# sisinflab/elliot

Measured on NVIDIA H100. Metric: bpr_triples_per_sec, higher is better.
Workload: dtype f32

## Files before the change

elliot_b200/csrc/bpr_train.cu:

```cuda
#include <cooperative_groups.h>
#include <cub/cub.cuh>
#include <stdlib.h>

#include <type_traits>

#include "bpr_update.cuh"

namespace eb {

struct HogwildParams {
    float *U, *V, *b;
    int ld;
    const int32_t *tu, *ti, *tj;
    int64_t n;
    BprHyper hp;
    double *loss;
    int32_t n_users, n_items;
    const int64_t *indptr;
    const int32_t *indices;
    uint64_t seed, first;
    int32_t *out_u, *out_i, *out_j;
    float *Vp[EB_MAX_PEERS], *bp[EB_MAX_PEERS];
    ShardMap shards;
    const uint32_t *filter;
    int filter_log2bits;
    const uint64_t *packed;
    int bits_u, bits_i;
    int no_item_updates;
    const int32_t *order;
};

__device__ __forceinline__ void sample_user(const HogwildParams &p, int64_t t, uint32_t (&r)[4], int &u, int64_t &beg, int &len) {
    Philox::gen(p.seed, p.first + (uint64_t)t, 0u, r);
    u = (int)bounded(r[0], (uint32_t)p.n_users);
    beg = __ldg(p.indptr + u);
    int64_t end = __ldg(p.indptr + u + 1);
    len = (int)(end - beg);
    uint32_t attempt = 0;
    while (len == 0 || len >= p.n_items) {
        Philox::gen(p.seed, p.first + (uint64_t)t, ++attempt | 0x80000000u, r);
        u = (int)bounded(r[0], (uint32_t)p.n_users);
        beg = __ldg(p.indptr + u); end = __ldg(p.indptr + u + 1); len = (int)(end - beg);
    }
}

__device__ __forceinline__ void sample_triple(const HogwildParams &p, int64_t t, int &u, int &i, int &j) {
    uint32_t r[4];
    int64_t beg;
    int len;
    sample_user(p, t, r, u, beg, len);
    uint32_t attempt = 0;
    const int32_t *row = p.indices + beg;
    int cand = (int)bounded(r[2], (uint32_t)p.n_items);
    const bool maybe = p.filter ? bloom_maybe(p.filter + ((int64_t)u << (p.filter_log2bits - 5)), p.filter_log2bits, (uint32_t)cand) : true;
    i = __ldg(row + bounded(r[1], (uint32_t)len));
    if (!maybe || !contains_sorted(row, len, cand)) { j = cand; return; }
    cand = (int)bounded(r[3], (uint32_t)p.n_items);
    attempt = 0;
    int q = 4;
    while (contains_sorted(row, len, cand) && attempt < 16u) {
        if (q == 4) { Philox::gen(p.seed, p.first + (uint64_t)t, ++attempt, r); q = 0; }
        cand = (int)bounded(r[q++], (uint32_t)p.n_items);
    }
    if (attempt >= 16u && contains_sorted(row, len, cand)) {
        Philox::gen(p.seed, p.first + (uint64_t)t, 0x40000000u, r);
        const uint32_t rank = bounded(r[0], (uint32_t)(p.n_items - len));
        int lo = 0, hi = len;
        while (lo < hi) {
            const int mid = (lo + hi) >> 1;
            if ((uint32_t)(__ldg(row + mid) - mid) > rank) hi = mid; else lo = mid + 1;
        }
        cand = (int)rank + lo;
    }
    j = cand;
}

template <bool SAMPLE>
__device__ __forceinline__ void fetch_triple(const HogwildParams &p, int64_t t, int &u, int &i, int &j) {
    if (SAMPLE) {
        sample_triple(p, t, u, i, j);
        if (p.out_u) { p.out_u[t] = u; p.out_i[t] = i; p.out_j[t] = j; }
    } else if (p.packed) {
        const uint64_t w = __ldg(p.packed + t);
        u = (int)(w & ((1ull << p.bits_u) - 1));
        i = (int)((w >> p.bits_u) & ((1ull << p.bits_i) - 1));
        j = (int)(w >> (p.bits_u + p.bits_i));
    } else {
        u = __ldg(p.tu + t); i = __ldg(p.ti + t); j = __ldg(p.tj + t);
    }
}

template <bool PEER>
__device__ __forceinline__ void item_row(const HogwildParams &p, int i, float *&row, float *&bias) {
    if constexpr (PEER) {
        int o, l;
        p.shards.locate(i, o, l);
        row = p.Vp[o] + (int64_t)l * p.ld; bias = p.bp[o] + l;
    } else {
        row = p.V + (int64_t)i * p.ld; bias = p.b + i;
    }
}

template <int VPL>
struct Rows {
    float4 u[VPL], vi[VPL], vj[VPL];
    float bi, bj;
};

template <int DP, bool SAMPLE, bool ATOMIC, bool PEER, bool ROUNDS = false>
__global__ void __launch_bounds__(256) bpr_hogwild_kernel(const HogwildParams p) {
    static_assert(!ROUNDS || (ATOMIC && !PEER), "deterministic rounds: local tables, atomic updates");
    constexpr int NV = DP / 4;
    constexpr int G = NV >= 32 ? 32 : NV;
    constexpr int VPL = NV / G;
    const int lane = threadIdx.x & 31;
    const int gl = lane % G;
    const int gbase = lane - gl;
    const int64_t warp_id = ((int64_t)blockIdx.x * blockDim.x + threadIdx.x) >> 5;
    const int64_t nwarps = ((int64_t)gridDim.x * blockDim.x) >> 5;
    const int64_t ld = p.ld;
    float loss_acc = 0.f;

    auto load_rows = [&](Rows<VPL> &r, int u, int i, int j) {
        if (u >= 0) {
            float *ri, *rj, *bi, *bj;
            item_row<PEER>(p, i, ri, bi); item_row<PEER>(p, j, rj, bj);
            const float4 *pu = reinterpret_cast<const float4 *>(p.U + (int64_t)u * ld);
            const float4 *pi = reinterpret_cast<const float4 *>(ri);
            const float4 *pj = reinterpret_cast<const float4 *>(rj);
#pragma unroll
            for (int v = 0; v < VPL; v++) {
                r.u[v] = pu[v * G + gl];
                r.vi[v] = PEER ? ld_sys_v4(pi + v * G + gl) : pi[v * G + gl];
                r.vj[v] = PEER ? ld_sys_v4(pj + v * G + gl) : pj[v * G + gl];
            }
            r.bi = *bi;
            r.bj = *bj;
        }
    };

    const int64_t n_tiles = (p.n + 31) / 32;
    const int64_t tile_end = ROUNDS ? (n_tiles + nwarps - 1) / nwarps * nwarps : n_tiles;
    for (int64_t tile = warp_id; tile < tile_end; tile += nwarps) {
        const int64_t t = tile * 32 + lane;
        int u = -1, i = 0, j = 0;
        if (t < p.n) fetch_triple<SAMPLE>(p, t, u, i, j);
        constexpr int UNR = G >= 4 ? 4 : G;
#pragma unroll 1
        for (int s0 = 0; s0 < G; s0 += UNR) {
            Rows<VPL> rw[UNR];
            int tu_[UNR], ti_[UNR], tj_[UNR];
#pragma unroll
            for (int q = 0; q < UNR; q++) {
                tu_[q] = __shfl_sync(0xffffffffu, u, gbase + s0 + q);
                ti_[q] = __shfl_sync(0xffffffffu, i, gbase + s0 + q);
                tj_[q] = __shfl_sync(0xffffffffu, j, gbase + s0 + q);
                load_rows(rw[q], tu_[q], ti_[q], tj_[q]);
            }
            if constexpr (ROUNDS) {
#pragma unroll
                for (int q = 0; q < UNR; q++) {
                    Rows<VPL> &cur = rw[q];
                    float part = 0.f;
                    if (tu_[q] >= 0) {
#pragma unroll
                        for (int v = 0; v < VPL; v++) part += bpr_partial_dot(cur.u[v], cur.vi[v], cur.vj[v]);
                    }
                    part = group_sum<G>(part);
                    if (tu_[q] >= 0) {
                        const float z = bpr_sigmoid_loss(part + (cur.bi - cur.bj), loss_acc, gl);
#pragma unroll
                        for (int v = 0; v < VPL; v++) {
                            float4 du, di, dj;
                            bpr_row_deltas(cur.u[v], cur.vi[v], cur.vj[v], z, p.hp, du, di, dj);
                            cur.u[v] = du; cur.vi[v] = di; cur.vj[v] = dj;
                        }
                        float dbi, dbj;
                        bpr_bias_deltas(z, cur.bi, cur.bj, p.hp, dbi, dbj);
                        cur.bi = dbi; cur.bj = dbj;
                    }
                }
                cooperative_groups::this_grid().sync();
#pragma unroll
                for (int q = 0; q < UNR; q++) {
                    if (tu_[q] < 0) continue;
                    float *pu = p.U + (int64_t)tu_[q] * ld, *pi, *pj, *pbi, *pbj;
                    item_row<PEER>(p, ti_[q], pi, pbi); item_row<PEER>(p, tj_[q], pj, pbj);
#pragma unroll
                    for (int v = 0; v < VPL; v++) {
                        const int e = (v * G + gl) * 4;
                        red_add_v4(pu + e, rw[q].u[v]);
                        red_add_v4(pi + e, rw[q].vi[v]);
                        red_add_v4(pj + e, rw[q].vj[v]);
                    }
                    if (gl == 0) { red_add_f32(pbi, rw[q].bi); red_add_f32(pbj, rw[q].bj); }
                }
                cooperative_groups::this_grid().sync();
                continue;
            }
#pragma unroll
            for (int q = 0; q < UNR; q++) {
                const Rows<VPL> &cur = rw[q];
                const int cu = tu_[q], ci = ti_[q], cj = tj_[q];
                float part = 0.f;
                if (cu >= 0) {
#pragma unroll
                    for (int v = 0; v < VPL; v++) part += bpr_partial_dot(cur.u[v], cur.vi[v], cur.vj[v]);
                }
                part = group_sum<G>(part);
                if (cu >= 0) {
                    const float z = bpr_sigmoid_loss(part + (cur.bi - cur.bj), loss_acc, gl);
                    float *pu = p.U + (int64_t)cu * ld, *pi, *pj, *pbi, *pbj;
                    item_row<PEER>(p, ci, pi, pbi); item_row<PEER>(p, cj, pj, pbj);
#pragma unroll
                    for (int v = 0; v < VPL; v++) {
                        const float4 a = cur.u[v], vi = cur.vi[v], vj = cur.vj[v];
                        float4 du, di, dj;
                        bpr_row_deltas(a, vi, vj, z, p.hp, du, di, dj);
                        const int e = (v * G + gl) * 4;
                        if (PEER) {
                            red_add_v4(pu + e, du);
                            if (!p.no_item_updates) {
                                red_add_v4_sys(pi + e, di);
                                red_add_v4_sys(pj + e, dj);
                            }
                        } else if (ATOMIC) {
                            red_add_v4(pu + e, du);
                            red_add_v4(pi + e, di);
                            red_add_v4(pj + e, dj);
                        } else {
                            *reinterpret_cast<float4 *>(pu + e) = make_float4(a.x + du.x, a.y + du.y, a.z + du.z, a.w + du.w);
                            *reinterpret_cast<float4 *>(pi + e) = make_float4(vi.x + di.x, vi.y + di.y, vi.z + di.z, vi.w + di.w);
                            *reinterpret_cast<float4 *>(pj + e) = make_float4(vj.x + dj.x, vj.y + dj.y, vj.z + dj.z, vj.w + dj.w);
                        }
                    }
                    if (gl == 0) {
                        float dbi, dbj;
                        bpr_bias_deltas(z, cur.bi, cur.bj, p.hp, dbi, dbj);
                        if (PEER) { red_add_f32_sys(pbi, dbi); red_add_f32_sys(pbj, dbj); }
                        else if (ATOMIC) { red_add_f32(pbi, dbi); red_add_f32(pbj, dbj); }
                        else { *pbi = cur.bi + dbi; *pbj = cur.bj + dbj; }
                    }
                }
            }
        }
    }
    if (p.loss) {
#pragma unroll
        for (int off = 16; off > 0; off >>= 1) loss_acc += __shfl_xor_sync(0xffffffffu, loss_acc, off);
        if (lane == 0 && loss_acc != 0.f) atomicAdd(p.loss, (double)loss_acc);
    }
}

__global__ void __launch_bounds__(256) user_key_kernel(const HogwildParams p, uint32_t *__restrict__ key, int32_t *__restrict__ val) {
    int64_t t = (int64_t)blockIdx.x * blockDim.x + threadIdx.x;
    const int64_t stride = (int64_t)gridDim.x * blockDim.x;
    for (; t < p.n; t += stride) {
        uint32_t r[4];
        int u, len;
        int64_t beg;
        sample_user(p, t, r, u, beg, len);
        key[t] = (uint32_t)u; val[t] = (int32_t)t;
    }
}

template <int DP, bool ATOMIC>
__global__ void __launch_bounds__(256) bpr_grouped_kernel(const HogwildParams p) {
    constexpr int NV = DP / 4;
    constexpr int G = NV >= 32 ? 32 : NV;
    constexpr int VPL = NV / G;
    constexpr int UNR = G >= 4 ? 4 : G;
    const int lane = threadIdx.x & 31;
    const int gl = lane % G;
    const int gbase = lane - gl;
    const int64_t warp_id = ((int64_t)blockIdx.x * blockDim.x + threadIdx.x) >> 5;
    const int64_t nwarps = ((int64_t)gridDim.x * blockDim.x) >> 5;
    const int64_t ld = p.ld;
    float loss_acc = 0.f;

    const int64_t n_tiles = (p.n + 31) / 32;
    for (int64_t tile = warp_id; tile < n_tiles; tile += nwarps) {
        const int64_t pos = tile * 32 + lane;
        int u = -1, i = 0, j = 0;
        if (pos < p.n) fetch_triple<true>(p, __ldg(p.order + pos), u, i, j);
        int cu = -1;
        float4 cur[VPL], acc[VPL];
        auto flush = [&]() {
            float *pu = p.U + (int64_t)cu * ld;
#pragma unroll
            for (int v = 0; v < VPL; v++) {
                float *e = pu + (v * G + gl) * 4;
                if (ATOMIC) red_add_v4(e, acc[v]);
                else *reinterpret_cast<float4 *>(e) = cur[v];
            }
        };
#pragma unroll 1
        for (int s0 = 0; s0 < G; s0 += UNR) {
            Rows<VPL> rw[UNR];
            int tu_[UNR], ti_[UNR], tj_[UNR];
#pragma unroll
            for (int q = 0; q < UNR; q++) {
                tu_[q] = __shfl_sync(0xffffffffu, u, gbase + s0 + q);
                ti_[q] = __shfl_sync(0xffffffffu, i, gbase + s0 + q);
                tj_[q] = __shfl_sync(0xffffffffu, j, gbase + s0 + q);
                if (tu_[q] >= 0) {
                    if (tu_[q] != (q == 0 ? cu : tu_[q - 1])) {
                        const float4 *pu = reinterpret_cast<const float4 *>(p.U + (int64_t)tu_[q] * ld);
#pragma unroll
                        for (int v = 0; v < VPL; v++) rw[q].u[v] = pu[v * G + gl];
                    }
                    const float4 *pi = reinterpret_cast<const float4 *>(p.V + (int64_t)ti_[q] * ld);
                    const float4 *pj = reinterpret_cast<const float4 *>(p.V + (int64_t)tj_[q] * ld);
#pragma unroll
                    for (int v = 0; v < VPL; v++) { rw[q].vi[v] = pi[v * G + gl]; rw[q].vj[v] = pj[v * G + gl]; }
                    rw[q].bi = p.b[ti_[q]];
                    rw[q].bj = p.b[tj_[q]];
                }
            }
#pragma unroll
            for (int q = 0; q < UNR; q++) {
                const Rows<VPL> &nx = rw[q];
                const int qu = tu_[q], qi = ti_[q], qj = tj_[q];
                const bool start = qu != cu;
                if (start) {
                    if (cu >= 0) flush();
                    cu = qu;
#pragma unroll
                    for (int v = 0; v < VPL; v++) cur[v] = nx.u[v];
                }
                float part = 0.f;
                if (qu >= 0) {
#pragma unroll
                    for (int v = 0; v < VPL; v++) part += bpr_partial_dot(cur[v], nx.vi[v], nx.vj[v]);
                }
                part = group_sum<G>(part);
                if (qu >= 0) {
                    const float z = bpr_sigmoid_loss(part + (nx.bi - nx.bj), loss_acc, gl);
                    float *pi = p.V + (int64_t)qi * ld, *pj = p.V + (int64_t)qj * ld;
#pragma unroll
                    for (int v = 0; v < VPL; v++) {
                        const float4 a = cur[v], vi = nx.vi[v], vj = nx.vj[v];
                        float4 du, di, dj;
                        bpr_row_deltas(a, vi, vj, z, p.hp, du, di, dj);
                        cur[v] = make_float4(a.x + du.x, a.y + du.y, a.z + du.z, a.w + du.w);
                        acc[v] = start ? du : make_float4(acc[v].x + du.x, acc[v].y + du.y, acc[v].z + du.z, acc[v].w + du.w);
                        const int e = (v * G + gl) * 4;
                        if (ATOMIC) {
                            red_add_v4(pi + e, di);
                            red_add_v4(pj + e, dj);
                        } else {
                            *reinterpret_cast<float4 *>(pi + e) = make_float4(vi.x + di.x, vi.y + di.y, vi.z + di.z, vi.w + di.w);
                            *reinterpret_cast<float4 *>(pj + e) = make_float4(vj.x + dj.x, vj.y + dj.y, vj.z + dj.z, vj.w + dj.w);
                        }
                    }
                    if (gl == 0) {
                        float dbi, dbj;
                        bpr_bias_deltas(z, nx.bi, nx.bj, p.hp, dbi, dbj);
                        if (ATOMIC) { red_add_f32(p.b + qi, dbi); red_add_f32(p.b + qj, dbj); }
                        else { p.b[qi] = nx.bi + dbi; p.b[qj] = nx.bj + dbj; }
                    }
                }
            }
        }
        if (cu >= 0) flush();
    }
    if (p.loss) {
#pragma unroll
        for (int off = 16; off > 0; off >>= 1) loss_acc += __shfl_xor_sync(0xffffffffu, loss_acc, off);
        if (lane == 0 && loss_acc != 0.f) atomicAdd(p.loss, (double)loss_acc);
    }
}

constexpr int STAGE_CHUNK_BYTES = 4096;
template <int DP, bool SAMPLE>
__global__ void __launch_bounds__(256) bpr_hogwild_stage_kernel(const HogwildParams p) {
    constexpr int NV = DP / 4;
    constexpr int G = NV >= 32 ? 32 : NV;
    constexpr int VPL = NV / G;
    constexpr int ROWB = DP * 4;
    constexpr int TT = STAGE_CHUNK_BYTES / ROWB;
    constexpr int NGRP = 32 / G;
    static_assert(TT >= NGRP && TT <= 32 && 32 % TT == 0, "chunk shape");
    extern __shared__ __align__(128) uint8_t stage_smem[];
    const int lane = threadIdx.x & 31, wib = threadIdx.x >> 5;
    const int gl = lane % G, grp = lane / G;
    uint8_t *wbuf = stage_smem + (size_t)wib * (TT * 3 * ROWB);
    uint64_t *bars = reinterpret_cast<uint64_t *>(stage_smem + (size_t)(blockDim.x >> 5) * (TT * 3 * ROWB));
    const uint32_t bar = (uint32_t)__cvta_generic_to_shared(bars + wib);
    const uint32_t wbuf_s = (uint32_t)__cvta_generic_to_shared(wbuf);
    if (lane == 0) {
        asm volatile("mbarrier.init.shared::cta.b64 [%0], %1;" ::"r"(bar), "r"(1) : "memory");
        asm volatile("fence.mbarrier_init.release.cluster;" ::: "memory");
    }
    __syncwarp();
    uint32_t phase = 0;
    const int64_t warp_id = ((int64_t)blockIdx.x * blockDim.x + threadIdx.x) >> 5;
    const int64_t nwarps = ((int64_t)gridDim.x * blockDim.x) >> 5;
    const int64_t ld = p.ld;
    float loss_acc = 0.f;

    for (int64_t tile = warp_id; tile * 32 < p.n; tile += nwarps) {
        const int64_t t = tile * 32 + lane;
        int u = -1, i = 0, j = 0;
        float bi = 0.f, bj = 0.f;
        float *pu = nullptr, *pi = nullptr, *pj = nullptr, *pbi = nullptr, *pbj = nullptr;
        if (t < p.n) {
            fetch_triple<SAMPLE>(p, t, u, i, j);
            pu = p.U + (int64_t)u * ld;
            item_row<true>(p, i, pi, pbi); item_row<true>(p, j, pj, pbj);
        }
        const bool valid = u >= 0;
#pragma unroll 1
        for (int c0 = 0; c0 < 32; c0 += TT) {
            const bool mine = valid && lane >= c0 && lane < c0 + TT;
            const uint32_t nmine = (uint32_t)__popc(__ballot_sync(0xffffffffu, mine));
            if (nmine == 0) continue;
            asm volatile("fence.proxy.async.shared::cta;" ::: "memory");
            __syncwarp();
            if (lane == 0)
                asm volatile("mbarrier.arrive.expect_tx.shared::cta.b64 _, [%0], %1;" ::"r"(bar), "r"(nmine * 3u * (uint32_t)ROWB) : "memory");
            __syncwarp();
            if (mine) {
                const uint32_t dst = wbuf_s + (uint32_t)(lane - c0) * (3u * ROWB);
                asm volatile("cp.async.bulk.shared::cluster.global.mbarrier::complete_tx::bytes [%0], [%1], %2, [%3];"
                             ::"r"(dst), "l"(pu), "r"(ROWB), "r"(bar) : "memory");
                asm volatile("cp.async.bulk.shared::cluster.global.mbarrier::complete_tx::bytes [%0], [%1], %2, [%3];"
                             ::"r"(dst + ROWB), "l"(pi), "r"(ROWB), "r"(bar) : "memory");
                asm volatile("cp.async.bulk.shared::cluster.global.mbarrier::complete_tx::bytes [%0], [%1], %2, [%3];"
                             ::"r"(dst + 2 * ROWB), "l"(pj), "r"(ROWB), "r"(bar) : "memory");
                bi = *pbi; bj = *pbj;
            }
            {
                uint32_t ok;
                do {
                    asm volatile("{\n\t.reg .pred q;\n\tmbarrier.try_wait.parity.shared::cta.b64 q, [%1], %2;\n\tselp.u32 %0, 1, 0, q;\n\t}"
                                 : "=r"(ok) : "r"(bar), "r"(phase) : "memory");
                } while (!ok);
                phase ^= 1;
            }
#pragma unroll 1
            for (int s = 0; s < TT; s += NGRP) {
                const int q = s + grp;
                const int src = c0 + q;
                const int cu = __shfl_sync(0xffffffffu, u, src), ci = __shfl_sync(0xffffffffu, i, src), cj = __shfl_sync(0xffffffffu, j, src);
                const float cbi = __shfl_sync(0xffffffffu, bi, src), cbj = __shfl_sync(0xffffffffu, bj, src);
                const bool on = cu >= 0;
                const float4 *su = reinterpret_cast<const float4 *>(wbuf + (size_t)q * (3 * ROWB));
                float4 a[VPL], vi[VPL], vj[VPL];
                float part = 0.f;
#pragma unroll
                for (int v = 0; v < VPL; v++) {
                    a[v] = su[v * G + gl]; vi[v] = su[NV + v * G + gl]; vj[v] = su[2 * NV + v * G + gl];
                    part += bpr_partial_dot(a[v], vi[v], vj[v]);
                }
                if (!on) part = 0.f;
                part = group_sum<G>(part);
                if (on) {
                    const float z = bpr_sigmoid_loss(part + (cbi - cbj), loss_acc, gl);
                    float *gu = p.U + (int64_t)cu * ld, *gi, *gj, *gbi, *gbj;
                    item_row<true>(p, ci, gi, gbi); item_row<true>(p, cj, gj, gbj);
#pragma unroll
                    for (int v = 0; v < VPL; v++) {
                        float4 du, di, dj;
                        bpr_row_deltas(a[v], vi[v], vj[v], z, p.hp, du, di, dj);
                        const int e = (v * G + gl) * 4;
                        red_add_v4(gu + e, du);
                        if (!p.no_item_updates) { red_add_v4_sys(gi + e, di); red_add_v4_sys(gj + e, dj); }
                    }
                    if (gl == 0) {
                        float dbi, dbj;
                        bpr_bias_deltas(z, cbi, cbj, p.hp, dbi, dbj);
                        red_add_f32_sys(gbi, dbi); red_add_f32_sys(gbj, dbj);
                    }
                }
            }
        }
    }
    if (p.loss) {
#pragma unroll
        for (int off = 16; off > 0; off >>= 1) loss_acc += __shfl_xor_sync(0xffffffffu, loss_acc, off);
        if (lane == 0 && loss_acc != 0.f) atomicAdd(p.loss, (double)loss_acc);
    }
}

static int persistent_grid(const void *kern, int smem, int64_t n, int reserve_sms, unsigned &grid) {
    int per_sm = 0;
    EB_CUDA(cudaOccupancyMaxActiveBlocksPerMultiprocessor(&per_sm, kern, 256, smem));
    if (per_sm < 1) per_sm = 1;
    const int64_t tiles = (n + 31) / 32;
    const int64_t want = (tiles + 7) / 8;
    int sms = sm_count() - reserve_sms;
    if (sms < 1) sms = 1;
    int64_t g = (int64_t)sms * per_sm;
    if (want < g) g = want;
    grid = (unsigned)(g < 1 ? 1 : g);
    return EB_OK;
}

template <int DP, bool SAMPLE>
static int launch_stage_t(const HogwildParams &p, int reserve_sms, cudaStream_t st) {
    constexpr int SMEM = 8 * 3 * STAGE_CHUNK_BYTES + 64;
    auto kern = bpr_hogwild_stage_kernel<DP, SAMPLE>;
    EB_CUDA(cudaFuncSetAttribute(kern, cudaFuncAttributeMaxDynamicSharedMemorySize, SMEM));
    unsigned grid;
    if (int rc = persistent_grid((const void *)kern, SMEM, p.n, reserve_sms, grid)) return rc;
    kern<<<grid, 256, SMEM, st>>>(p);
    EB_CUDA(cudaGetLastError());
    return EB_OK;
}

__global__ void __launch_bounds__(256) bloom_build_kernel(const int64_t *__restrict__ indptr, const int32_t *__restrict__ indices,
                                                          int32_t n_users, int log2bits, uint32_t *__restrict__ out) {
    const int lane = threadIdx.x & 31;
    int64_t w = ((int64_t)blockIdx.x * blockDim.x + threadIdx.x) >> 5;
    const int64_t nw = ((int64_t)gridDim.x * blockDim.x) >> 5;
    const int words = 1 << (log2bits - 5);
    for (; w < n_users; w += nw) {
        uint32_t *f = out + w * words;
        for (int k = lane; k < words; k += 32) f[k] = 0u;
        __syncwarp();
        const int64_t beg = indptr[w], end = indptr[w + 1];
        for (int64_t e = beg + lane; e < end; e += 32) {
            uint32_t a, b;
            bloom_bits((uint32_t)indices[e], log2bits, a, b);
            atomicOr(f + (a >> 5), 1u << (a & 31));
            atomicOr(f + (b >> 5), 1u << (b & 31));
        }
        __syncwarp();
    }
}

__global__ void __launch_bounds__(256) philox_sample_kernel(const HogwildParams p) {
    int64_t t = (int64_t)blockIdx.x * blockDim.x + threadIdx.x;
    const int64_t stride = (int64_t)gridDim.x * blockDim.x;
    for (; t < p.n; t += stride) {
        int u, i, j;
        sample_triple(p, t, u, i, j);
        p.out_u[t] = u; p.out_i[t] = i; p.out_j[t] = j;
    }
}

__global__ void __launch_bounds__(256) pointwise_sample_kernel(const HogwildParams p, float *__restrict__ out_label) {
    int64_t t = (int64_t)blockIdx.x * blockDim.x + threadIdx.x;
    const int64_t stride = (int64_t)gridDim.x * blockDim.x;
    for (; t < p.n; t += stride) {
        int u, i, j;
        sample_triple(p, t, u, i, j);
        uint32_t r[4];
        Philox::gen(p.seed, p.first + (uint64_t)t, 0x20000000u, r);
        const bool pos = (r[0] >> 31) != 0;
        p.out_u[t] = u; p.out_i[t] = pos ? i : j; out_label[t] = pos ? 1.f : 0.f;
    }
}

template <int DP, bool SAMPLE, bool ATOMIC, bool PEER, bool ROUNDS>
static int launch_hogwild_t(const HogwildParams &p, int reserve_sms, cudaStream_t st) {
    auto kern = bpr_hogwild_kernel<DP, SAMPLE, ATOMIC, PEER, ROUNDS>;
    unsigned grid;
    if (int rc = persistent_grid((const void *)kern, 0, p.n, reserve_sms, grid)) return rc;
    if (ROUNDS) {
        void *args[] = {const_cast<HogwildParams *>(&p)};
        EB_CUDA(cudaLaunchCooperativeKernel((const void *)kern, dim3(grid), dim3(256), args, 0, st));
    } else {
        kern<<<grid, 256, 0, st>>>(p);
    }
    EB_CUDA(cudaGetLastError());
    return EB_OK;
}

template <int... DPS, class F>
static int with_stride(int dp, const char *strides, F &&f) {
    int rc = EB_OK;
    const bool found = ((dp == DPS && (rc = f(std::integral_constant<int, DPS>{}), true)) || ...);
    return found ? rc : set_err(EB_ERR_ARG, "row stride ld=%d must be one of %s", dp, strides);
}

static void item_table_l2_window(const HogwildParams &p, cudaStream_t st) {
    static const int env = [] { const char *e = getenv("EB_L2_PERSIST"); return e ? atoi(e) : 0; }();
    if (!env || !p.V) return;
    static int max_persist = -1, max_window = 0;
    if (max_persist < 0) {
        int dev = 0; cudaGetDevice(&dev);
        cudaDeviceGetAttribute(&max_persist, cudaDevAttrMaxPersistingL2CacheSize, dev);
        cudaDeviceGetAttribute(&max_window, cudaDevAttrMaxAccessPolicyWindowSize, dev);
    }
    const size_t bytes = (size_t)p.n_items * (size_t)p.ld * sizeof(float);
    if (max_persist <= 0 || bytes > (size_t)max_persist || bytes > (size_t)max_window) return;
    static size_t carved = 0;
    if (carved != bytes) { cudaDeviceSetLimit(cudaLimitPersistingL2CacheSize, bytes); carved = bytes; }
    cudaStreamAttrValue attr{};
    attr.accessPolicyWindow.base_ptr = (void *)p.V;
    attr.accessPolicyWindow.num_bytes = bytes;
    attr.accessPolicyWindow.hitRatio = 1.0f;
    attr.accessPolicyWindow.hitProp = cudaAccessPropertyPersisting;
    attr.accessPolicyWindow.missProp = env == 2 ? cudaAccessPropertyNormal : cudaAccessPropertyStreaming;
    cudaStreamSetAttribute(st, cudaStreamAttributeAccessPolicyWindow, &attr);
}

template <int DP, bool ATOMIC>
static int launch_grouped_t(const HogwildParams &p, int reserve_sms, cudaStream_t st) {
    auto kern = bpr_grouped_kernel<DP, ATOMIC>;
    unsigned grid;
    if (int rc = persistent_grid((const void *)kern, 0, p.n, reserve_sms, grid)) return rc;
    kern<<<grid, 256, 0, st>>>(p);
    EB_CUDA(cudaGetLastError());
    return EB_OK;
}

static inline size_t align_up(size_t x, size_t a = 256) { return (x + a - 1) / a * a; }

static int bits_for(uint64_t v) { int b = 1; while ((v >> b) != 0) b++; return b; }

constexpr int64_t GROUP_MAX = (int64_t)INT32_MAX;

struct GroupLayout {
    size_t key_a, key_b, val_a, val_b, cub, cub_bytes, total;
};

static GroupLayout group_layout(int64_t n, int32_t n_users) {
    const int64_t m = n < GROUP_MAX ? n : GROUP_MAX;
    GroupLayout L;
    size_t off = 0;
    L.key_a = off; off += align_up(sizeof(uint32_t) * (size_t)m);
    L.key_b = off; off += align_up(sizeof(uint32_t) * (size_t)m);
    L.val_a = off; off += align_up(sizeof(int32_t) * (size_t)m);
    L.val_b = off; off += align_up(sizeof(int32_t) * (size_t)m);
    cub::DoubleBuffer<uint32_t> keys(nullptr, nullptr);
    cub::DoubleBuffer<int32_t> vals(nullptr, nullptr);
    size_t cb = 0;
    cub::DeviceRadixSort::SortPairs(nullptr, cb, keys, vals, (int)m, 0, bits_for((uint64_t)n_users));
    L.cub_bytes = cb;
    L.cub = off; off += align_up(cb);
    L.total = off;
    return L;
}

template <int DP, bool ATOMIC>
static int launch_grouped(HogwildParams p, int reserve, char *ws, const GroupLayout &L, cudaStream_t st) {
    const int ubits = bits_for((uint64_t)p.n_users);
    const int64_t n = p.n;
    const uint64_t first = p.first;
    int32_t *out_u = p.out_u, *out_i = p.out_i, *out_j = p.out_j;
    int sms = sm_count() - reserve;
    if (sms < 1) sms = 1;
    for (int64_t c0 = 0; c0 < n; c0 += GROUP_MAX) {
        p.n = n - c0 < GROUP_MAX ? n - c0 : GROUP_MAX;
        p.first = first + (uint64_t)c0;
        if (out_u) { p.out_u = out_u + c0; p.out_i = out_i + c0; p.out_j = out_j + c0; }
        cub::DoubleBuffer<uint32_t> keys((uint32_t *)(ws + L.key_a), (uint32_t *)(ws + L.key_b));
        cub::DoubleBuffer<int32_t> vals((int32_t *)(ws + L.val_a), (int32_t *)(ws + L.val_b));
        int64_t grid = (p.n + 255) / 256;
        if (grid > (int64_t)sms * 8) grid = (int64_t)sms * 8;
        user_key_kernel<<<(unsigned)grid, 256, 0, st>>>(p, keys.Current(), vals.Current());
        EB_CUDA(cudaGetLastError());
        size_t cb = L.cub_bytes;
        EB_CUDA(cub::DeviceRadixSort::SortPairs(ws + L.cub, cb, keys, vals, (int)p.n, 0, ubits, st));
        p.order = vals.Current();
        if (int rc = launch_grouped_t<DP, ATOMIC>(p, reserve, st)) return rc;
    }
    return EB_OK;
}

template <bool SAMPLE>
static int launch_hogwild(const HogwildParams &p, int dp, int flags, cudaStream_t st, void *ws = nullptr, size_t ws_bytes = 0) {
    const bool atomic = !(flags & 1);
    const bool rounds = (flags & 64) != 0;
    const int reserve = (flags >> 8) & 0xff;
    EB_ARG(!(flags & 32), "the shared-memory-staged kernel exists for sharded item tables only");
    EB_ARG(atomic || !rounds, "deterministic rounds run with atomic updates");
    if constexpr (SAMPLE) {
        if (!rounds) {
            const GroupLayout L = group_layout(p.n, p.n_users);
            if (!ws || ws_bytes < L.total) return set_err(EB_ERR_WORKSPACE, "workspace %zu < required %zu", ws ? ws_bytes : 0, L.total);
            return with_stride<8, 16, 32, 64, 128, 256>(dp, "8,16,32,64,128,256 floats", [&](auto dpc) {
                constexpr int DP = decltype(dpc)::value;
                item_table_l2_window(p, st);
                return atomic ? launch_grouped<DP, true>(p, reserve, (char *)ws, L, st)
                              : launch_grouped<DP, false>(p, reserve, (char *)ws, L, st);
            });
        }
    }
    item_table_l2_window(p, st);
    return with_stride<8, 16, 32, 64, 128, 256>(dp, "8,16,32,64,128,256 floats", [&](auto dpc) {
        constexpr int DP = decltype(dpc)::value;
        if constexpr (!SAMPLE) {
            if (!rounds) return atomic ? launch_hogwild_t<DP, false, true, false, false>(p, reserve, st)
                                       : launch_hogwild_t<DP, false, false, false, false>(p, reserve, st);
        }
        return launch_hogwild_t<DP, SAMPLE, true, false, true>(p, reserve, st);
    });
}

template <bool SAMPLE>
static int launch_hogwild_peer(const HogwildParams &p, int dp, int flags, cudaStream_t st) {
    const int reserve = (flags >> 8) & 0xff;
    EB_ARG(!(flags & 64), "deterministic rounds exist for local tables only (other GPUs update peer rows concurrently)");
    const bool stage = !(flags & (1 | 16));
    return with_stride<32, 64, 128>(dp, "32,64,128 floats for sharded item tables", [&](auto dpc) {
        constexpr int DP = decltype(dpc)::value;
        return stage ? launch_stage_t<DP, SAMPLE>(p, reserve, st) : launch_hogwild_t<DP, SAMPLE, true, true, false>(p, reserve, st);
    });
}

static int fill_peer(HogwildParams &p, float *const *V_shards, float *const *b_shards, int n_shards, int32_t shard_rows,
                     int32_t n_items) {
    EB_ARG(V_shards && b_shards && n_shards >= 1 && n_shards <= EB_MAX_PEERS, "1 <= n_shards <= %d", EB_MAX_PEERS);
    EB_ARG(shard_rows >= 1 && (int64_t)shard_rows * n_shards >= n_items, "shards do not cover the item range");
    for (int s = 0; s < n_shards; s++) {
        EB_ARG(V_shards[s] && b_shards[s] && ((uintptr_t)V_shards[s] % 16) == 0, "null / misaligned shard pointer %d", s);
        p.Vp[s] = V_shards[s]; p.bp[s] = b_shards[s];
    }
    for (int s = n_shards; s < EB_MAX_PEERS; s++) { p.Vp[s] = V_shards[0]; p.bp[s] = b_shards[0]; }
    p.shards = shard_map(shard_rows);
    return EB_OK;
}

static int check_tables(const void *U, const void *V, const void *b, int d, int ld) {
    EB_ARG(U && V && b, "null table pointer");
    EB_ARG(d >= 1 && ld >= d, "need 1 <= d <= ld (d=%d ld=%d)", d, ld);
    EB_ARG(((uintptr_t)U % 16) == 0 && ((uintptr_t)V % 16) == 0, "tables must be 16-byte aligned");
    return EB_OK;
}

struct ExactParams {
    double *U, *V, *b;
    int d, ld;
    const int32_t *tu, *ti, *tj;
    const int32_t *ku, *ki, *kj;
    int32_t *cntU, *cntI, *ticket;
    int64_t n;
    double lr, reg_u, reg_b, reg_pos, reg_neg;
    double *loss;
};

__device__ __forceinline__ int ld_acquire(const int32_t *p) {
    int v;
    asm volatile("ld.acquire.gpu.global.s32 %0, [%1];" : "=r"(v) : "l"(p) : "memory");
    return v;
}
__device__ __forceinline__ void st_release(int32_t *p, int v) {
    asm volatile("st.release.gpu.global.s32 [%0], %1;" ::"l"(p), "r"(v) : "memory");
}

template <int NE>
__global__ void __launch_bounds__(128) bpr_exact_kernel(const ExactParams p) {
    const int lane = threadIdx.x & 31;
    double loss_acc = 0.0;
    for (;;) {
        int t = 0;
        if (lane == 0) t = atomicAdd(p.ticket, 1);
        t = __shfl_sync(0xffffffffu, t, 0);
        if (t >= p.n) break;
        const int u = __ldg(p.tu + t), i = __ldg(p.ti + t), j = __ldg(p.tj + t);
        const int wu = __ldg(p.ku + t), wi = __ldg(p.ki + t), wj = __ldg(p.kj + t);
        int32_t *cu = p.cntU + u, *ci = p.cntI + i, *cj = p.cntI + j;
        {
            unsigned ns = 8;
            for (;;) {
                const bool ready = (ld_acquire(cu) == wu) & (ld_acquire(ci) == wi) & (ld_acquire(cj) == wj);
                if (__all_sync(0xffffffffu, ready)) break;
                __nanosleep(ns);
                if (ns < 128) ns <<= 1;
            }
        }
        double *pu = p.U + (int64_t)u * p.ld, *pi = p.V + (int64_t)i * p.ld, *pj = p.V + (int64_t)j * p.ld;
        double a[NE], vi[NE], vj[NE];
        double xi = 0.0, xj = 0.0;
#pragma unroll
        for (int e = 0; e < NE; e++) {
            const int k = lane + 32 * e;
            a[e] = 0.0; vi[e] = 0.0; vj[e] = 0.0;
            if (k < p.d) {
                a[e] = __ldcg(pu + k); vi[e] = __ldcg(pi + k); vj[e] = __ldcg(pj + k);
                xi = __dadd_rn(xi, __dmul_rn(a[e], vi[e]));
                xj = __dadd_rn(xj, __dmul_rn(a[e], vj[e]));
            }
        }
#pragma unroll
        for (int off = 16; off > 0; off >>= 1) {
            xi = __dadd_rn(xi, __shfl_xor_sync(0xffffffffu, xi, off));
            xj = __dadd_rn(xj, __shfl_xor_sync(0xffffffffu, xj, off));
        }
        const double bi = __ldcg(p.b + i), bj = __ldcg(p.b + j);
        xi = __dadd_rn(xi, bi);
        xj = __dadd_rn(xj, bj);
        const double x = __dadd_rn(xi, -xj);
        const double z = 1.0 / (1.0 + exp(x));
        const double sp = (x > 0) ? log1p(exp(-x)) : (-x + log1p(exp(x)));
        loss_acc += (lane == 0) ? sp : 0.0;
#pragma unroll
        for (int e = 0; e < NE; e++) {
            const int k = lane + 32 * e;
            const double un = __dadd_rn(
                a[e], __dmul_rn(p.lr, __dadd_rn(__dmul_rn(__dadd_rn(vi[e], -vj[e]), z), -__dmul_rn(p.reg_u, a[e]))));
            const double uz = __dmul_rn(un, z);
            const double in_ = __dadd_rn(vi[e], __dmul_rn(p.lr, __dadd_rn(uz, -__dmul_rn(p.reg_pos, vi[e]))));
            const double jn = __dadd_rn(vj[e], __dmul_rn(p.lr, __dadd_rn(-uz, -__dmul_rn(p.reg_neg, vj[e]))));
            if (k < p.d) { __stcg(pu + k, un); __stcg(pi + k, in_); __stcg(pj + k, jn); }
        }
        const double bin = __dadd_rn(bi, __dmul_rn(p.lr, __dadd_rn(z, -__dmul_rn(p.reg_b, bi))));
        const double bjn = __dadd_rn(bj, __dmul_rn(p.lr, __dadd_rn(-z, -__dmul_rn(p.reg_b, bj))));
        if (lane == 0) { __stcg(p.b + i, bin); __stcg(p.b + j, bjn); }
        __threadfence();
        const unsigned done = __ballot_sync(0xffffffffu, true);
        if (done == 0xffffffffu) {
            if (lane == 0) st_release(cu, wu + 1);
            else if (lane == 1) st_release(ci, wi + 1);
            else if (lane == 2) st_release(cj, wj + 1);
        }
    }
    if (p.loss && lane == 0 && loss_acc != 0.0) atomicAdd(p.loss, loss_acc);
}

__global__ void make_keys_kernel(const int32_t *tu, const int32_t *ti, const int32_t *tj, int64_t n, int ebits,
                                 uint64_t *keysU, uint64_t *keysI, int32_t n_users, int32_t n_items, int32_t *status) {
    int64_t t = (int64_t)blockIdx.x * blockDim.x + threadIdx.x;
    if (t >= n) return;
    const uint32_t uu = (uint32_t)tu[t], ii = (uint32_t)ti[t], jj = (uint32_t)tj[t];
    if (ii == jj) atomicOr(status, 1);
    if (uu >= (uint32_t)n_users || ii >= (uint32_t)n_items || jj >= (uint32_t)n_items) { atomicOr(status, 2); return; }
    keysU[t] = ((uint64_t)(uint32_t)tu[t] << ebits) | (uint64_t)t;
    keysI[2 * t] = ((uint64_t)(uint32_t)ti[t] << ebits) | (uint64_t)(2 * t);
    keysI[2 * t + 1] = ((uint64_t)(uint32_t)tj[t] << ebits) | (uint64_t)(2 * t + 1);
}

__global__ void ranks_kernel(const uint64_t *keys, int64_t m, int ebits, int is_items, int32_t *ka, int32_t *kb) {
    int64_t pos = (int64_t)blockIdx.x * blockDim.x + threadIdx.x;
    if (pos >= m) return;
    const uint64_t key = keys[pos];
    const uint64_t first = (key >> ebits) << ebits;
    int64_t lo = 0, hi = pos;
    while (lo < hi) {
        int64_t mid = (lo + hi) >> 1;
        if (keys[mid] < first) lo = mid + 1; else hi = mid;
    }
    const int32_t rank = (int32_t)(pos - lo);
    const uint64_t ev = key & ((1ull << ebits) - 1);
    if (!is_items) ka[ev] = rank;
    else if (ev & 1) kb[ev >> 1] = rank;
    else ka[ev >> 1] = rank;
}

struct ExactLayout {
    size_t keys_in, keys_out, ku, ki, kj, cnt, cub, total, cub_bytes;
};

static ExactLayout exact_layout(int64_t n, int32_t n_users, int32_t n_items) {
    ExactLayout L;
    size_t off = 0;
    L.keys_in = off; off += align_up(sizeof(uint64_t) * 3 * (size_t)n);
    L.keys_out = off; off += align_up(sizeof(uint64_t) * 3 * (size_t)n);
    L.ku = off; off += align_up(sizeof(int32_t) * (size_t)n);
    L.ki = off; off += align_up(sizeof(int32_t) * (size_t)n);
    L.kj = off; off += align_up(sizeof(int32_t) * (size_t)n);
    L.cnt = off; off += align_up(sizeof(int32_t) * ((size_t)n_users + (size_t)n_items + 64));
    size_t cb = 0;
    cub::DeviceRadixSort::SortKeys(nullptr, cb, (const uint64_t *)nullptr, (uint64_t *)nullptr, (int64_t)(2 * n), 0, 64);
    L.cub_bytes = cb;
    L.cub = off; off += align_up(cb);
    L.total = off;
    return L;
}

}

using namespace eb;

extern "C" int eb_bpr_step_f32(float *U, float *V, float *item_bias, int d, int ld, const int32_t *tu,
                               const int32_t *ti, const int32_t *tj, int64_t n, float lr, float reg_u, float reg_b,
                               float reg_pos, float reg_neg, double *loss, int flags, void *stream) {
    if (int rc = check_tables(U, V, item_bias, d, ld)) return rc;
    EB_ARG(n >= 0, "n < 0");
    if (n == 0) return EB_OK;
    EB_ARG(tu && ti && tj, "null triple arrays");
    HogwildParams p{};
    p.U = U; p.V = V; p.b = item_bias; p.ld = ld; p.tu = tu; p.ti = ti; p.tj = tj; p.n = n;
    p.hp = {lr, reg_u, reg_b, reg_pos, reg_neg}; p.loss = loss;
    return launch_hogwild<false>(p, ld, flags, (cudaStream_t)stream);
}

static int set_filter(HogwildParams &p, const uint32_t *filter, int filter_words) {
    if (!filter) return EB_OK;
    EB_ARG(filter_words >= 1 && filter_words <= 1024 && (filter_words & (filter_words - 1)) == 0,
           "filter_words must be a power of two in [1, 1024] (got %d)", filter_words);
    int lb = 5;
    while ((1 << (lb - 5)) < filter_words) lb++;
    p.filter = filter; p.filter_log2bits = lb;
    return EB_OK;
}

extern "C" int eb_bloom_build(const int64_t *csr_indptr, const int32_t *csr_indices, int32_t n_users, int filter_words,
                              uint32_t *out, void *stream) {
    EB_ARG(csr_indptr && csr_indices && out && n_users >= 1, "bad argument");
    HogwildParams p{};
    if (int rc = set_filter(p, out, filter_words)) return rc;
    int64_t grid = ((int64_t)n_users * 32 + 255) / 256;
    const int64_t cap = (int64_t)sm_count() * 8;
    if (grid > cap) grid = cap;
    bloom_build_kernel<<<(unsigned)grid, 256, 0, (cudaStream_t)stream>>>(csr_indptr, csr_indices, n_users, p.filter_log2bits, out);
    EB_CUDA(cudaGetLastError());
    return EB_OK;
}

extern "C" int eb_bpr_step_sampled_f32(float *U, float *V, float *item_bias, int d, int ld, int32_t n_users,
                                       int32_t n_items, const int64_t *csr_indptr, const int32_t *csr_indices,
                                       int64_t n, uint64_t seed, uint64_t first_triple, float lr, float reg_u,
                                       float reg_b, float reg_pos, float reg_neg, double *loss, int32_t *out_u,
                                       int32_t *out_i, int32_t *out_j, void *workspace, size_t workspace_bytes, int flags,
                                       void *stream) {
    return eb_bpr_step_sampled_filter_f32(U, V, item_bias, d, ld, n_users, n_items, csr_indptr, csr_indices, nullptr, 0, n, seed,
                                          first_triple, lr, reg_u, reg_b, reg_pos, reg_neg, loss, out_u, out_i, out_j, workspace,
                                          workspace_bytes, flags, stream);
}

extern "C" size_t eb_bpr_step_sampled_workspace_bytes(int64_t n, int32_t n_users) {
    if (n <= 0 || n_users <= 0) return 256;
    return group_layout(n, n_users).total;
}

extern "C" int eb_bpr_step_sampled_filter_f32(float *U, float *V, float *item_bias, int d, int ld, int32_t n_users,
                                              int32_t n_items, const int64_t *csr_indptr, const int32_t *csr_indices,
                                              const uint32_t *filter, int filter_words, int64_t n, uint64_t seed,
                                              uint64_t first_triple, float lr, float reg_u, float reg_b, float reg_pos,
                                              float reg_neg, double *loss, int32_t *out_u, int32_t *out_i, int32_t *out_j,
                                              void *workspace, size_t workspace_bytes, int flags, void *stream) {
    if (int rc = check_tables(U, V, item_bias, d, ld)) return rc;
    EB_ARG(n >= 0 && n_users > 0 && n_items > 1, "bad sizes");
    EB_ARG(csr_indptr && csr_indices, "null CSR");
    EB_ARG((!out_u && !out_i && !out_j) || (out_u && out_i && out_j), "out_u/out_i/out_j: all or none");
    if (n == 0) return EB_OK;
    HogwildParams p{};
    p.U = U; p.V = V; p.b = item_bias; p.ld = ld; p.n = n;
    p.hp = {lr, reg_u, reg_b, reg_pos, reg_neg}; p.loss = loss;
    p.n_users = n_users; p.n_items = n_items; p.indptr = csr_indptr; p.indices = csr_indices;
    p.seed = seed; p.first = first_triple; p.out_u = out_u; p.out_i = out_i; p.out_j = out_j;
    if (int rc = set_filter(p, filter, filter_words)) return rc;
    return launch_hogwild<true>(p, ld, flags, (cudaStream_t)stream, workspace, workspace_bytes);
}

extern "C" int eb_bpr_step_peer_f32(float *U, float *const *V_shards, float *const *b_shards, int n_shards, int32_t shard_rows,
                                    int d, int ld, int32_t n_items, const int32_t *tu, const int32_t *ti, const int32_t *tj, int64_t n,
                                    float lr, float reg_u, float reg_b, float reg_pos, float reg_neg, double *loss, int flags,
                                    void *stream) {
    EB_ARG(U && d >= 1 && ld >= d && ((uintptr_t)U % 16) == 0, "bad user table");
    EB_ARG(n >= 0, "n < 0");
    HogwildParams p{};
    if (int rc = fill_peer(p, V_shards, b_shards, n_shards, shard_rows, n_items)) return rc;
    if (n == 0) return EB_OK;
    EB_ARG(tu && ti && tj, "null triple arrays");
    p.U = U; p.ld = ld; p.tu = tu; p.ti = ti; p.tj = tj; p.n = n;
    p.hp = {lr, reg_u, reg_b, reg_pos, reg_neg}; p.loss = loss;
    return launch_hogwild_peer<false>(p, ld, flags, (cudaStream_t)stream);
}

extern "C" int eb_bpr_step_sampled_peer_f32(float *U, float *const *V_shards, float *const *b_shards, int n_shards, int32_t shard_rows,
                                            int d, int ld, int32_t n_users, int32_t n_items, const int64_t *csr_indptr,
                                            const int32_t *csr_indices, const uint32_t *filter, int filter_words, int64_t n,
                                            uint64_t seed, uint64_t first_triple, float lr,
                                            float reg_u, float reg_b, float reg_pos, float reg_neg, double *loss, int32_t *out_u,
                                            int32_t *out_i, int32_t *out_j, int flags, void *stream) {
    EB_ARG(U && d >= 1 && ld >= d && ((uintptr_t)U % 16) == 0, "bad user table");
    EB_ARG(n >= 0 && n_users > 0 && n_items > 1, "bad sizes");
    EB_ARG(csr_indptr && csr_indices, "null CSR");
    EB_ARG((!out_u && !out_i && !out_j) || (out_u && out_i && out_j), "out_u/out_i/out_j: all or none");
    HogwildParams p{};
    if (int rc = fill_peer(p, V_shards, b_shards, n_shards, shard_rows, n_items)) return rc;
    if (n == 0) return EB_OK;
    p.U = U; p.ld = ld; p.n = n;
    p.hp = {lr, reg_u, reg_b, reg_pos, reg_neg}; p.loss = loss;
    p.n_users = n_users; p.n_items = n_items; p.indptr = csr_indptr; p.indices = csr_indices;
    p.seed = seed; p.first = first_triple; p.out_u = out_u; p.out_i = out_i; p.out_j = out_j;
    p.no_item_updates = (flags >> 2) & 1;
    if (int rc = set_filter(p, filter, filter_words)) return rc;
    return launch_hogwild_peer<true>(p, ld, flags, (cudaStream_t)stream);
}

extern "C" int eb_bpr_sample_philox(int32_t n_users, int32_t n_items, const int64_t *csr_indptr,
                                    const int32_t *csr_indices, int64_t n, uint64_t seed, uint64_t first_triple,
                                    int32_t *out_u, int32_t *out_i, int32_t *out_j, void *stream) {
    return eb_bpr_sample_philox_filter(n_users, n_items, csr_indptr, csr_indices, nullptr, 0, n, seed, first_triple, out_u, out_i,
                                       out_j, stream);
// ... 138 lines not shown
```

Measured before the change: 2.297 billion.

## Stage user-row tiles in shared memory with ticket-scheduled tile blocks

Replaces the warp-grouped BPR kernel with a block-per-user-tile kernel. Each block takes a user tile from an atomic ticket counter and loads that tile's user rows and indptr into shared memory. It then updates the user rows in shared memory across all triples for the tile, split across thread groups at user boundaries, and writes the tile back once. A new kernel computes tile offsets from the sorted keys. This is meant to cut global traffic on user rows and the per-user flush atomics. The cost is extra shared memory, block-level syncs, and load imbalance when tiles are skewed. It also writes user rows back non-atomically, which assumes tiles are owned by a single block.

```diff
diff --git a/elliot_b200/csrc/bpr_train.cu b/elliot_b200/csrc/bpr_train.cu
--- a/elliot_b200/csrc/bpr_train.cu
+++ b/elliot_b200/csrc/bpr_train.cu
@@ -27,7 +27,10 @@
     const uint64_t *packed;
     int bits_u, bits_i;
     int no_item_updates;
-    const int32_t *order;
+    const int32_t *order, *tile_off;
+    int32_t *tile_ticket;
+    int64_t n_tiles;
+    int tile_bits;
 };
 
 __device__ __forceinline__ void sample_user(const HogwildParams &p, int64_t t, uint32_t (&r)[4], int &u, int64_t &beg, int &len) {
@@ -44,11 +47,8 @@
     }
 }
 
-__device__ __forceinline__ void sample_triple(const HogwildParams &p, int64_t t, int &u, int &i, int &j) {
-    uint32_t r[4];
-    int64_t beg;
-    int len;
-    sample_user(p, t, r, u, beg, len);
+__device__ __forceinline__ void sample_items(const HogwildParams &p, int64_t t, uint32_t (&r)[4], int u, int64_t beg, int len, int &i,
+                                             int &j) {
     uint32_t attempt = 0;
     const int32_t *row = p.indices + beg;
     int cand = (int)bounded(r[2], (uint32_t)p.n_items);
@@ -73,6 +73,27 @@
         cand = (int)rank + lo;
     }
     j = cand;
+}
+
+__device__ __forceinline__ void sample_triple(const HogwildParams &p, int64_t t, int &u, int &i, int &j) {
+    uint32_t r[4];
+    int64_t beg;
+    int len;
+    sample_user(p, t, r, u, beg, len);
+    sample_items(p, t, r, u, beg, len, i, j);
+}
+
+__device__ __forceinline__ void sample_in_tile(const HogwildParams &p, int64_t t, int64_t u0, int nu, const int64_t *s_ptr, int &u,
+                                               int &i, int &j) {
+    uint32_t r[4];
+    Philox::gen(p.seed, p.first + (uint64_t)t, 0u, r);
+    u = (int)bounded(r[0], (uint32_t)p.n_users);
+    const int64_t ul = (int64_t)u - u0;
+    int64_t beg = 0;
+    int len = 0;
+    if (ul >= 0 && ul < nu) { beg = s_ptr[ul]; len = (int)(s_ptr[ul + 1] - beg); }
+    if (len == 0 || len >= p.n_items) sample_user(p, t, r, u, beg, len);
+    sample_items(p, t, r, u, beg, len, i, j);
 }
 
 template <bool SAMPLE>
@@ -252,6 +273,13 @@
     }
 }
 
+constexpr int TILE_THREADS = 256;
+constexpr int TILE_CAP = 2048;
+constexpr int TILE_ROW_BYTES = 32768;
+constexpr int tile_users(int DP) { return TILE_ROW_BYTES / (DP * 4) < 256 ? TILE_ROW_BYTES / (DP * 4) : 256; }
+constexpr int TILE_MIN_USERS = tile_users(256);
+constexpr int tile_smem_bytes(int DP) { return tile_users(DP) * DP * 4 + (tile_users(DP) + 1) * 8 + TILE_CAP * (2 * 4 + 2); }
+
 __global__ void __launch_bounds__(256) user_key_kernel(const HogwildParams p, uint32_t *__restrict__ key, int32_t *__restrict__ val) {
     int64_t t = (int64_t)blockIdx.x * blockDim.x + threadIdx.x;
     const int64_t stride = (int64_t)gridDim.x * blockDim.x;
@@ -264,105 +292,131 @@
     }
 }
 
+__global__ void __launch_bounds__(256) tile_bounds_kernel(const uint32_t *__restrict__ key, int64_t n, int tile_bits, int64_t n_tiles,
+                                                          int32_t *__restrict__ tile_off, int32_t *__restrict__ ticket) {
+    int64_t pos = (int64_t)blockIdx.x * blockDim.x + threadIdx.x;
+    const int64_t stride = (int64_t)gridDim.x * blockDim.x;
+    if (pos == 0) *ticket = 0;
+    for (; pos <= n; pos += stride) {
+        const int64_t prev = pos > 0 ? (int64_t)(key[pos - 1] >> tile_bits) : -1;
+        const int64_t cur = pos < n ? (int64_t)(key[pos] >> tile_bits) : n_tiles;
+        for (int64_t k = prev + 1; k <= cur; k++) tile_off[k] = (int32_t)pos;
+    }
+}
+
 template <int DP, bool ATOMIC>
-__global__ void __launch_bounds__(256) bpr_grouped_kernel(const HogwildParams p) {
+__global__ void __launch_bounds__(TILE_THREADS, 2) bpr_tile_kernel(const HogwildParams p) {
     constexpr int NV = DP / 4;
     constexpr int G = NV >= 32 ? 32 : NV;
     constexpr int VPL = NV / G;
     constexpr int UNR = G >= 4 ? 4 : G;
-    const int lane = threadIdx.x & 31;
-    const int gl = lane % G;
-    const int gbase = lane - gl;
-    const int64_t warp_id = ((int64_t)blockIdx.x * blockDim.x + threadIdx.x) >> 5;
-    const int64_t nwarps = ((int64_t)gridDim.x * blockDim.x) >> 5;
-    const int64_t ld = p.ld;
+    constexpr int T = tile_users(DP);
+    constexpr int NG = TILE_THREADS / G;
+    extern __shared__ __align__(16) uint8_t tile_smem[];
+    float4 *rows = reinterpret_cast<float4 *>(tile_smem);
+    int64_t *s_ptr = reinterpret_cast<int64_t *>(rows + T * NV);
+    int32_t *e_i = reinterpret_cast<int32_t *>(s_ptr + T + 1), *e_j = e_i + TILE_CAP;
+    uint16_t *e_u = reinterpret_cast<uint16_t *>(e_j + TILE_CAP);
+    __shared__ int64_t s_tile;
+    const int tid = threadIdx.x, lane = tid & 31, gl = lane % G, grp = tid / G;
     float loss_acc = 0.f;
 
-    const int64_t n_tiles = (p.n + 31) / 32;
-    for (int64_t tile = warp_id; tile < n_tiles; tile += nwarps) {
-        const int64_t pos = tile * 32 + lane;
-        int u = -1, i = 0, j = 0;
-        if (pos < p.n) fetch_triple<true>(p, __ldg(p.order + pos), u, i, j);
-        int cu = -1;
-        float4 cur[VPL], acc[VPL];
-        auto flush = [&]() {
-            float *pu = p.U + (int64_t)cu * ld;
-#pragma unroll
-            for (int v = 0; v < VPL; v++) {
-                float *e = pu + (v * G + gl) * 4;
-                if (ATOMIC) red_add_v4(e, acc[v]);
-                else *reinterpret_cast<float4 *>(e) = cur[v];
+    for (;;) {
+        __syncthreads();
+        if (tid == 0) s_tile = atomicAdd(p.tile_ticket, 1);
+        __syncthreads();
+        const int64_t tile = s_tile;
+        if (tile >= p.n_tiles) break;
+        const int beg = p.tile_off[tile], end = p.tile_off[tile + 1];
+        if (beg == end) continue;
+        const int64_t u0 = tile * T;
+        const int nu = (int)(p.n_users - u0 < T ? p.n_users - u0 : T);
+        float4 *gU = reinterpret_cast<float4 *>(p.U + u0 * DP);
+        for (int k = tid; k < nu * NV; k += TILE_THREADS) rows[k] = gU[k];
+        for (int k = tid; k <= nu; k += TILE_THREADS) s_ptr[k] = __ldg(p.indptr + u0 + k);
+        __syncthreads();
+
+        for (int c0 = beg; c0 < end; c0 += TILE_CAP) {
+            const int m = end - c0 < TILE_CAP ? end - c0 : TILE_CAP;
+            for (int k = tid; k < m; k += TILE_THREADS) {
+                const int t = __ldg(p.order + c0 + k);
+                int u, i, j;
+                sample_in_tile(p, t, u0, nu, s_ptr, u, i, j);
+                if (p.out_u) { p.out_u[t] = u; p.out_i[t] = i; p.out_j[t] = j; }
+                e_i[k] = i; e_j[k] = j; e_u[k] = (uint16_t)(u - u0);
             }
-        };
+            __syncthreads();
+            auto boundary = [&](int a) {
+                while (a > 0 && a < m && e_u[a] == e_u[a - 1]) a++;
+                return a;
+            };
+            const int lo = boundary(grp * m / NG), len = boundary((grp + 1) * m / NG) - lo;
+            const int wlen = (int)__reduce_max_sync(0xffffffffu, (unsigned)len);
 #pragma unroll 1
-        for (int s0 = 0; s0 < G; s0 += UNR) {
-            Rows<VPL> rw[UNR];
-            int tu_[UNR], ti_[UNR], tj_[UNR];
-#pragma unroll
-            for (int q = 0; q < UNR; q++) {
-                tu_[q] = __shfl_sync(0xffffffffu, u, gbase + s0 + q);
-                ti_[q] = __shfl_sync(0xffffffffu, i, gbase + s0 + q);
-                tj_[q] = __shfl_sync(0xffffffffu, j, gbase + s0 + q);
-                if (tu_[q] >= 0) {
-                    if (tu_[q] != (q == 0 ? cu : tu_[q - 1])) {
-                        const float4 *pu = reinterpret_cast<const float4 *>(p.U + (int64_t)tu_[q] * ld);
-#pragma unroll
-                        for (int v = 0; v < VPL; v++) rw[q].u[v] = pu[v * G + gl];
+            for (int s0 = 0; s0 < wlen; s0 += UNR) {
+                float4 vi[UNR][VPL], vj[UNR][VPL];
+                float bi[UNR], bj[UNR];
+                int qu[UNR], qi[UNR], qj[UNR];
+#pragma unroll
+                for (int q = 0; q < UNR; q++) {
+                    qu[q] = -1; qi[q] = 0; qj[q] = 0; bi[q] = 0.f; bj[q] = 0.f;
+                    if (s0 + q < len) {
+                        const int k = lo + s0 + q;
+                        qu[q] = e_u[k]; qi[q] = e_i[k]; qj[q] = e_j[k];
+                        const float4 *pi = reinterpret_cast<const float4 *>(p.V + (int64_t)qi[q] * DP);
+                        const float4 *pj = reinterpret_cast<const float4 *>(p.V + (int64_t)qj[q] * DP);
+#pragma unroll
+                        for (int v = 0; v < VPL; v++) { vi[q][v] = pi[v * G + gl]; vj[q][v] = pj[v * G + gl]; }
+                        bi[q] = p.b[qi[q]];
+                        bj[q] = p.b[qj[q]];
                     }
-                    const float4 *pi = reinterpret_cast<const float4 *>(p.V + (int64_t)ti_[q] * ld);
-                    const float4 *pj = reinterpret_cast<const float4 *>(p.V + (int64_t)tj_[q] * ld);
-#pragma unroll
-                    for (int v = 0; v < VPL; v++) { rw[q].vi[v] = pi[v * G + gl]; rw[q].vj[v] = pj[v * G + gl]; }
-                    rw[q].bi = p.b[ti_[q]];
-                    rw[q].bj = p.b[tj_[q]];
                 }
-            }
-#pragma unroll
-            for (int q = 0; q < UNR; q++) {
-                const Rows<VPL> &nx = rw[q];
-                const int qu = tu_[q], qi = ti_[q], qj = tj_[q];
-                const bool start = qu != cu;
-                if (start) {
-                    if (cu >= 0) flush();
-                    cu = qu;
-#pragma unroll
-                    for (int v = 0; v < VPL; v++) cur[v] = nx.u[v];
-                }
-                float part = 0.f;
-                if (qu >= 0) {
-#pragma unroll
-                    for (int v = 0; v < VPL; v++) part += bpr_partial_dot(cur[v], nx.vi[v], nx.vj[v]);
-                }
-                part = group_sum<G>(part);
-                if (qu >= 0) {
-                    const float z = bpr_sigmoid_loss(part + (nx.bi - nx.bj), loss_acc, gl);
-                    float *pi = p.V + (int64_t)qi * ld, *pj = p.V + (int64_t)qj * ld;
-#pragma unroll
-                    for (int v = 0; v < VPL; v++) {
-                        const float4 a = cur[v], vi = nx.vi[v], vj = nx.vj[v];
-                        float4 du, di, dj;
-                        bpr_row_deltas(a, vi, vj, z, p.hp, du, di, dj);
-                        cur[v] = make_float4(a.x + du.x, a.y + du.y, a.z + du.z, a.w + du.w);
-                        acc[v] = start ? du : make_float4(acc[v].x + du.x, acc[v].y + du.y, acc[v].z + du.z, acc[v].w + du.w);
-                        const int e = (v * G + gl) * 4;
-                        if (ATOMIC) {
-                            red_add_v4(pi + e, di);
-                            red_add_v4(pj + e, dj);
-                        } else {
-                            *reinterpret_cast<float4 *>(pi + e) = make_float4(vi.x + di.x, vi.y + di.y, vi.z + di.z, vi.w + di.w);
-                            *reinterpret_cast<float4 *>(pj + e) = make_float4(vj.x + dj.x, vj.y + dj.y, vj.z + dj.z, vj.w + dj.w);
+#pragma unroll
+                for (int q = 0; q < UNR; q++) {
+                    const bool on = qu[q] >= 0;
+                    float4 *ur = rows + (on ? qu[q] : 0) * NV;
+                    float4 a[VPL];
+                    float part = 0.f;
+                    if (on) {
+#pragma unroll
+                        for (int v = 0; v < VPL; v++) {
+                            a[v] = ur[v * G + gl];
+                            part += bpr_partial_dot(a[v], vi[q][v], vj[q][v]);
                         }
                     }
-                    if (gl == 0) {
-                        float dbi, dbj;
-                        bpr_bias_deltas(z, nx.bi, nx.bj, p.hp, dbi, dbj);
-                        if (ATOMIC) { red_add_f32(p.b + qi, dbi); red_add_f32(p.b + qj, dbj); }
-                        else { p.b[qi] = nx.bi + dbi; p.b[qj] = nx.bj + dbj; }
+                    part = group_sum<G>(part);
+                    if (on) {
+                        const float z = bpr_sigmoid_loss(part + (bi[q] - bj[q]), loss_acc, gl);
+                        float *pi = p.V + (int64_t)qi[q] * DP, *pj = p.V + (int64_t)qj[q] * DP;
+#pragma unroll
+                        for (int v = 0; v < VPL; v++) {
+                            float4 du, di, dj;
+                            const float4 x = vi[q][v], y = vj[q][v];
+                            bpr_row_deltas(a[v], x, y, z, p.hp, du, di, dj);
+                            const float4 c = a[v];
+                            ur[v * G + gl] = ATOMIC ? make_float4(__fadd_rn(c.x, du.x), __fadd_rn(c.y, du.y), __fadd_rn(c.z, du.z), __fadd_rn(c.w, du.w))
+                                                    : make_float4(c.x + du.x, c.y + du.y, c.z + du.z, c.w + du.w);
+                            const int e = (v * G + gl) * 4;
+                            if (ATOMIC) {
+                                red_add_v4(pi + e, di);
+                                red_add_v4(pj + e, dj);
+                            } else {
+                                *reinterpret_cast<float4 *>(pi + e) = make_float4(x.x + di.x, x.y + di.y, x.z + di.z, x.w + di.w);
+                                *reinterpret_cast<float4 *>(pj + e) = make_float4(y.x + dj.x, y.y + dj.y, y.z + dj.z, y.w + dj.w);
+                            }
+                        }
+                        if (gl == 0) {
+                            float dbi, dbj;
+                            bpr_bias_deltas(z, bi[q], bj[q], p.hp, dbi, dbj);
+                            if (ATOMIC) { red_add_f32(p.b + qi[q], dbi); red_add_f32(p.b + qj[q], dbj); }
+                            else { p.b[qi[q]] = bi[q] + dbi; p.b[qj[q]] = bj[q] + dbj; }
+                        }
                     }
                 }
             }
-        }
-        if (cu >= 0) flush();
+            __syncthreads();
+        }
+        for (int k = tid; k < nu * NV; k += TILE_THREADS) gU[k] = rows[k];
     }
     if (p.loss) {
 #pragma unroll
@@ -598,11 +652,18 @@
 }
 
 template <int DP, bool ATOMIC>
-static int launch_grouped_t(const HogwildParams &p, int reserve_sms, cudaStream_t st) {
-    auto kern = bpr_grouped_kernel<DP, ATOMIC>;
-    unsigned grid;
-    if (int rc = persistent_grid((const void *)kern, 0, p.n, reserve_sms, grid)) return rc;
-    kern<<<grid, 256, 0, st>>>(p);
+static int launch_tile_t(const HogwildParams &p, int reserve_sms, cudaStream_t st) {
+    constexpr int SMEM = tile_smem_bytes(DP);
+    auto kern = bpr_tile_kernel<DP, ATOMIC>;
+    EB_CUDA(cudaFuncSetAttribute(kern, cudaFuncAttributeMaxDynamicSharedMemorySize, SMEM));
+    int per_sm = 0;
+    EB_CUDA(cudaOccupancyMaxActiveBlocksPerMultiprocessor(&per_sm, kern, TILE_THREADS, SMEM));
+    if (per_sm < 1) per_sm = 1;
+    int sms = sm_count() - reserve_sms;
+    if (sms < 1) sms = 1;
+    int64_t grid = (int64_t)sms * per_sm;
+    if (grid > p.n_tiles) grid = p.n_tiles;
+    kern<<<(unsigned)grid, TILE_THREADS, SMEM, st>>>(p);
     EB_CUDA(cudaGetLastError());
     return EB_OK;
 }
@@ -614,7 +675,7 @@
 constexpr int64_t GROUP_MAX = (int64_t)INT32_MAX;
 
 struct GroupLayout {
-    size_t key_a, key_b, val_a, val_b, cub, cub_bytes, total;
+    size_t key_a, key_b, val_a, val_b, tile_off, ticket, cub, cub_bytes, total;
 };
 
 static GroupLayout group_layout(int64_t n, int32_t n_users) {
@@ -625,6 +686,8 @@
     L.key_b = off; off += align_up(sizeof(uint32_t) * (size_t)m);
     L.val_a = off; off += align_up(sizeof(int32_t) * (size_t)m);
     L.val_b = off; off += align_up(sizeof(int32_t) * (size_t)m);
+    L.tile_off = off; off += align_up(sizeof(int32_t) * ((size_t)((n_users + (int64_t)TILE_MIN_USERS - 1) / TILE_MIN_USERS) + 1));
+    L.ticket = off; off += align_up(sizeof(int32_t));
     cub::DoubleBuffer<uint32_t> keys(nullptr, nullptr);
     cub::DoubleBuffer<int32_t> vals(nullptr, nullptr);
     size_t cb = 0;
@@ -636,13 +699,18 @@
 }
 
 template <int DP, bool ATOMIC>
-static int launch_grouped(HogwildParams p, int reserve, char *ws, const GroupLayout &L, cudaStream_t st) {
+static int launch_tiled(HogwildParams p, int reserve, char *ws, const GroupLayout &L, cudaStream_t st) {
     const int ubits = bits_for((uint64_t)p.n_users);
     const int64_t n = p.n;
     const uint64_t first = p.first;
     int32_t *out_u = p.out_u, *out_i = p.out_i, *out_j = p.out_j;
     int sms = sm_count() - reserve;
     if (sms < 1) sms = 1;
+    constexpr int T = tile_users(DP);
+    p.tile_bits = bits_for((uint64_t)T) - 1;
+    p.n_tiles = ((int64_t)p.n_users + T - 1) / T;
+    p.tile_off = (const int32_t *)(ws + L.tile_off);
+    p.tile_ticket = (int32_t *)(ws + L.ticket);
     for (int64_t c0 = 0; c0 < n; c0 += GROUP_MAX) {
         p.n = n - c0 < GROUP_MAX ? n - c0 : GROUP_MAX;
         p.first = first + (uint64_t)c0;
@@ -656,7 +724,10 @@
         size_t cb = L.cub_bytes;
         EB_CUDA(cub::DeviceRadixSort::SortPairs(ws + L.cub, cb, keys, vals, (int)p.n, 0, ubits, st));
         p.order = vals.Current();
-        if (int rc = launch_grouped_t<DP, ATOMIC>(p, reserve, st)) return rc;
+        tile_bounds_kernel<<<(unsigned)grid, 256, 0, st>>>(keys.Current(), p.n, p.tile_bits, p.n_tiles, (int32_t *)(ws + L.tile_off),
+                                                           p.tile_ticket);
+        EB_CUDA(cudaGetLastError());
+        if (int rc = launch_tile_t<DP, ATOMIC>(p, reserve, st)) return rc;
     }
     return EB_OK;
 }
@@ -675,8 +746,8 @@
             return with_stride<8, 16, 32, 64, 128, 256>(dp, "8,16,32,64,128,256 floats", [&](auto dpc) {
                 constexpr int DP = decltype(dpc)::value;
                 item_table_l2_window(p, st);
-                return atomic ? launch_grouped<DP, true>(p, reserve, (char *)ws, L, st)
-                              : launch_grouped<DP, false>(p, reserve, (char *)ws, L, st);
+                return atomic ? launch_tiled<DP, true>(p, reserve, (char *)ws, L, st)
+                              : launch_tiled<DP, false>(p, reserve, (char *)ws, L, st);
             });
         }
     }
```

After: 2.360 billion (median of 6 runs). 1.03x the previous value.
